# stateSpaceRobotics/pointcloud_obstacle_processing

Hardware: NVIDIA B200
Metric: points/sec per B200 job (HDL-64 120k-point frames: crop + 0.1 m voxel + RANSAC ground removal + Euclidean clustering + centroid/radius) (higher is better)
Workload: dtype f32

## Files before the change

pointcloud_obstacle_processing_b200/csrc/det_math.cuh:

```cuda
#pragma once
#include "common.cuh"

namespace pcop {

#define PCOP_INV_ODD_TABLE                                                                                            \
  {1.0 / 1.0,  1.0 / 3.0,  1.0 / 5.0,  1.0 / 7.0,  1.0 / 9.0,  1.0 / 11.0, 1.0 / 13.0, 1.0 / 15.0, 1.0 / 17.0, 1.0 / 19.0, \
   1.0 / 21.0, 1.0 / 23.0, 1.0 / 25.0, 1.0 / 27.0, 1.0 / 29.0}

__device__ inline double det_log(double x) {
  int e;
  double m = frexp(x, &e);
  if (m < 0.70710678118654752440) {
    m = dmul(m, 2.0);
    e -= 1;
  }
  const double s = ddiv(dsub(m, 1.0), dadd(m, 1.0));
  const double z = dmul(s, s);
  const double INV_ODD[15] = PCOP_INV_ODD_TABLE;
  double p = INV_ODD[14];
#pragma unroll
  for (int k = 13; k >= 0; --k) p = dadd(dmul(p, z), INV_ODD[k]);
  return dadd(dmul((double)e, 0.69314718055994530942), dmul(dmul(2.0, s), p));
}

__device__ inline double det_atan01(double t) {
  const double ATAN_K[5] = {0.0, 0.24497866312686415417, 0.46364760900080611621, 0.64350110879328438680,
                            0.78539816339744830962};
  const int k = (int)dadd(dmul(4.0, t), 0.5);
  const double c = dmul((double)k, 0.25);
  const double u = ddiv(dsub(t, c), dadd(1.0, dmul(t, c)));
  const double z = dmul(u, u);
  const double INV_ODD[15] = PCOP_INV_ODD_TABLE;
  double q = INV_ODD[10];
#pragma unroll
  for (int j = 9; j >= 0; --j) q = dsub(INV_ODD[j], dmul(z, q));
  return dadd(ATAN_K[k], dmul(u, q));
}

__device__ inline double det_atan2_ypos(double y, double x) {
  const double PI = 3.14159265358979323846, PI_2 = 1.57079632679489661923;
  if (y == 0.0) return (x >= 0.0) ? 0.0 : PI;
  if (x == 0.0) return PI_2;
  const double ax = fabs(x);
  double a;
  if (y <= ax) a = det_atan01(ddiv(y, ax));
  else a = dsub(PI_2, det_atan01(ddiv(ax, y)));
  return (x > 0.0) ? a : dsub(PI, a);
}

__device__ inline double det_sin(double x) {
  const double F[11] = {1.0,
                        1.0 / 6.0,
                        1.0 / 120.0,
                        1.0 / 5040.0,
                        1.0 / 362880.0,
                        1.0 / 39916800.0,
                        1.0 / 6227020800.0,
                        1.0 / 1307674368000.0,
                        1.0 / 355687428096000.0,
                        1.0 / 121645100408832000.0,
                        1.0 / 51090942171709440000.0};
  const double z = dmul(x, x);
  double p = 1.0 / 25852016738884976640000.0;
  for (int j = 10; j >= 0; --j) p = dsub(F[j], dmul(z, p));
  return dmul(x, p);
}

__device__ inline double det_cos(double x) {
  const double F[11] = {1.0,
                        1.0 / 2.0,
                        1.0 / 24.0,
                        1.0 / 720.0,
                        1.0 / 40320.0,
                        1.0 / 3628800.0,
                        1.0 / 479001600.0,
                        1.0 / 87178291200.0,
                        1.0 / 20922789888000.0,
                        1.0 / 6402373705728000.0,
                        1.0 / 2432902008176640000.0};
  const double z = dmul(x, x);
  double p = 1.0 / 1124000727777607680000.0;
  for (int j = 10; j >= 0; --j) p = dsub(F[j], dmul(z, p));
  return p;
}

__device__ inline double det_asin(double q) {
  if (q != q || fabs(q) > 1.0) return __longlong_as_double(0x7ff8000000000000ll);
  const double a = fabs(q);
  const double x = __dsqrt_rn(dmul(dsub(1.0, a), dadd(1.0, a)));
  const double r = det_atan2_ypos(a, x);
  return (q < 0.0) ? -r : r;
}

__device__ inline double det_tan(double x) { return ddiv(det_sin(x), det_cos(x)); }

}
```

pointcloud_obstacle_processing_b200/csrc/stage_plane.cu:

```cuda
#include "det_math.cuh"
#include <cstdio>
#include "internal.cuh"
#include "primitives.cuh"

namespace pcop {
#ifdef PCOP_PLANE_DEBUG_CLK
__device__ long long g_plane_loop_clk[16];
#define PL_CLK(k)                                                                  \
  do {                                                                             \
    if (blockIdx.y == 0 && rank == 0 && threadIdx.x == 0) g_plane_loop_clk[k] = clock64(); \
  } while (0)
#else
#define PL_CLK(k) \
  do {            \
  } while (0)
#endif

namespace {

constexpr int MAP_CAP = RNG_TABLE + 8;
constexpr double kHalfPi = 1.57079632679489661923;

__device__ __forceinline__ const float4* cur_cloud(const PlaneFrame& P, const float4* in, size_t in_stride,
                                                   float4* const* buf, int f, int cap) {
  return (P.cur < 0) ? (in + (size_t)f * in_stride) : (buf[P.cur] + (size_t)f * cap);
}

struct BufPair {
  float4* p[2];
  int* s[2];
};

__device__ bool model_valid(const PlaneConst& pc, const float4 co) {
  if (!(pc.eps_angle > 0.0)) return true;
  if (pc.eps_angle >= kHalfPi) return true;
  const double nx = co.x, ny = co.y, nz = co.z;
  const double dot = dadd(dadd(dmul(nx, pc.axis[0]), dmul(ny, pc.axis[1])), dmul(nz, pc.axis[2]));
  const double nn = __dsqrt_rn(dadd(dadd(dmul(nx, nx), dmul(ny, ny)), dmul(nz, nz)));
  const double na = __dsqrt_rn(dadd(dadd(dmul(pc.axis[0], pc.axis[0]), dmul(pc.axis[1], pc.axis[1])),
                                    dmul(pc.axis[2], pc.axis[2])));
  const double cosang = ddiv(fabs(dot), dmul(nn, na));
  return !(cosang < pc.cos_eps);
}

__device__ __forceinline__ bool collinear_ratio_test(const float4 p0, const float4 p1, const float4 p2) {
  const float ax = fdiv(fsub(p1.x, p0.x), fsub(p2.x, p0.x));
  const float ay = fdiv(fsub(p1.y, p0.y), fsub(p2.y, p0.y));
  const float az = fdiv(fsub(p1.z, p0.z), fsub(p2.z, p0.z));
  return (ax == ay) && (az == ay);
}

__device__ float4 compute_model(const float4 p0, const float4 p1, const float4 p2) {
  const float ax = fsub(p1.x, p0.x), ay = fsub(p1.y, p0.y), az = fsub(p1.z, p0.z);
  const float bx = fsub(p2.x, p0.x), by = fsub(p2.y, p0.y), bz = fsub(p2.z, p0.z);
  float nx = fsub(fmul(ay, bz), fmul(az, by));
  float ny = fsub(fmul(az, bx), fmul(ax, bz));
  float nz = fsub(fmul(ax, by), fmul(ay, bx));
  const float norm = __fsqrt_rn(fadd(fadd(fmul(nx, nx), fmul(ny, ny)), fmul(nz, nz)));
  nx = fdiv(nx, norm);
  ny = fdiv(ny, norm);
  nz = fdiv(nz, norm);
  const float d = -fadd(fadd(fmul(nx, p0.x), fmul(ny, p0.y)), fmul(nz, p0.z));
  return make_float4(nx, ny, nz, d);
}

__global__ void k_plane_init(PlaneFrame* __restrict__ pf, const int* __restrict__ n_in, double keep_fraction,
                             int* __restrict__ n_active, int* __restrict__ n_in_copy, int B) {
  const int f = blockIdx.x * blockDim.x + threadIdx.x;
  if (f >= B) return;
  PlaneFrame& P = pf[f];
  const int n = n_in[f];
  if (n_in_copy) n_in_copy[f] = n;
  P.cur = -1;
  P.nr_points = n;
  P.n = n;
  P.n_passes = 0;
  P.n_hyp = 0;
  P.gen_end = 0;
  P.best = -1;
  P.model_ok = 0;
  P.need_more = 0;
  P.n_inliers_last = 0;
  P.coeff_sel = make_float4(0.f, 0.f, 0.f, 0.f);
  P.coeff_ref = make_float4(0.f, 0.f, 0.f, 0.f);
  for (int k = 0; k < PCOP_MAX_PLANE_PASSES_RECORDED; ++k) {
    P.pass_points[k] = 0;
    P.pass_inliers[k] = 0;
    P.pass_coeff[k] = make_float4(0.f, 0.f, 0.f, 0.f);
  }
  P.active = ((double)n > dmul(keep_fraction, (double)n)) ? 1 : 0;
  if (P.active) atomicAdd(n_active, 1);
  atomicMax(n_active + 1, n);
  atomicAdd(n_active + 2, n);
}

// ... 171 lines not shown
        if (!gen_end) gen_end = 1;
        break;
      }
      const float4 co = compute_model(p0, p1, p2);
      if (lane == 0) {
        hyp[nh] = co;
        hyp_valid[nh] = model_valid(pc, co) ? 1 : 0;
      }
      ++nh;
    }
  }
  __syncwarp();
  nh_out = nh;
  gen_end_out = gen_end;
}

__global__ void __launch_bounds__(32)
    k_plane_gen(PlaneFrame* __restrict__ pf, const float4* __restrict__ in, size_t in_stride, BufPair bp,
                const int* __restrict__ rng, PlaneConst pc, uint32_t* __restrict__ warnings, int cap) {
  const int f = blockIdx.x;
  PlaneFrame& P = pf[f];
  if (!P.active) return;
  const int lane = threadIdx.x;
  __shared__ GenScratch G;
  int nh, gen_end;
  plane_gen_warp(cur_cloud(P, in, in_stride, bp.p, f, cap), P.n, rng, pc, G, P.hyp, P.hyp_valid, nh, gen_end);
  if (lane == 0) {
    P.n_hyp = nh;
    P.gen_end = gen_end;
    if (gen_end == 2) atomicOr(&warnings[f], (uint32_t)PCOP_WARN_RNG_TABLE_EXHAUSTED);
  }
  for (int h = lane; h < MAX_HYP; h += 32) P.counts[h] = 0;
}

__global__ void __launch_bounds__(CT_THREADS)
    k_plane_score(PlaneFrame* __restrict__ pf, const float4* __restrict__ in, size_t in_stride, BufPair bp, float thr,
                  int cap, int h_begin, int h_end, int second_phase) {
  const int f = blockIdx.y;
  PlaneFrame& P = pf[f];
  if (!P.active) return;
  if (second_phase && !P.need_more) return;
  const int n = P.n;
  if (blockIdx.x * CT_TILE >= n) return;
  const int nh = min(P.n_hyp, h_end);
  if (nh <= h_begin) return;
  __shared__ float4 hyp[MAX_HYP];
  __shared__ int cnt[MAX_HYP];
  if (threadIdx.x < MAX_HYP) {
    const float qnan = __uint_as_float(0x7fc00000u);
    hyp[threadIdx.x] = (threadIdx.x < nh) ? P.hyp[threadIdx.x] : make_float4(qnan, qnan, qnan, qnan);
    cnt[threadIdx.x] = 0;
  }
  __syncthreads();
  const float4* pts = cur_cloud(P, in, in_stride, bp.p, f, cap);
  const int lane = lane_id();
  for (int tile = blockIdx.x; tile * CT_TILE < n; tile += gridDim.x) {
  float4 p[CT_ITEMS];
#pragma unroll
  for (int k = 0; k < CT_ITEMS; ++k) {
    const int i = ct_index(tile, k);
    const float qnan = __uint_as_float(0x7fc00000u);
    p[k] = (i < n) ? __ldg(pts + i) : make_float4(qnan, qnan, qnan, qnan);
  }
  for (int h0 = h_begin; h0 < nh; h0 += 8) {
    int c[8];
#pragma unroll
    for (int j = 0; j < 8; ++j) {
      c[j] = 0;
      const float4 co = hyp[h0 + j];
#pragma unroll
      for (int k = 0; k < CT_ITEMS; ++k) c[j] += (plane_dist(co, p[k].x, p[k].y, p[k].z) < thr) ? 1 : 0;
    }
#pragma unroll
    for (int j = 0; j < 8; ++j) {
      const int s = __reduce_add_sync(FULL, c[j]);
      if (lane == 0 && s) atomicAdd(&cnt[h0 + j], s);
    }
  }
  }
  __syncthreads();
  if (threadIdx.x >= h_begin && threadIdx.x < nh && cnt[threadIdx.x]) atomicAdd(&P.counts[threadIdx.x], cnt[threadIdx.x]);
}

template <class CountFn>
__device__ __forceinline__ bool plane_select_replay(const PlaneConst& pc, double log_probability, int n, int nh, int navail,
                                                    const int* hyp_valid, CountFn count, int& sel_out) {
  const double one_over_indices = ddiv(1.0, (double)n);
  const double eps = 2.220446049250313e-16;
  int best = -2147483647;
  int sel = -1;
  double k = 1.0;
  for (int h = 0; h < nh; ++h) {
    if (!((double)h < k)) break;
    if (h >= navail) return true;
    const int c = hyp_valid[h] ? count(h) : 0;
    if (c > best) {
      best = c;
      sel = h;
      const double w = dmul((double)best, one_over_indices);
      double p_no = dsub(1.0, dmul(dmul(w, w), w));
      p_no = (eps < p_no) ? p_no : eps;
      p_no = (p_no < dsub(1.0, eps)) ? p_no : dsub(1.0, eps);
      k = ddiv(log_probability, det_log(p_no));
    }
    if (h + 1 > pc.max_iterations) break;
  }
  sel_out = sel;
  return false;
}

__global__ void k_plane_select(PlaneFrame* __restrict__ pf, PlaneConst pc, int B, int navail, int second_phase) {
  const int f = blockIdx.x * blockDim.x + threadIdx.x;
  if (f >= B) return;
  PlaneFrame& P = pf[f];
  if (!P.active) return;
  if (second_phase && !P.need_more) return;
  P.need_more = 0;
  int sel = -1;
  const int* counts = P.counts;
  if (plane_select_replay(pc, det_log(dsub(1.0, pc.probability)), P.n, P.n_hyp, navail, P.hyp_valid,
                          [counts](int h) { return counts[h]; }, sel)) {
    P.need_more = 1;
    return;
  }
  P.best = sel;
  P.model_ok = (sel >= 0 && P.hyp_valid[sel]) ? 1 : 0;
  P.coeff_sel = (sel >= 0) ? P.hyp[sel] : make_float4(0.f, 0.f, 0.f, 0.f);
  P.coeff_ref = P.coeff_sel;
}

template <int MINB>
__global__ void __launch_bounds__(256, MINB)
    k_plane_moments(const PlaneFrame* __restrict__ pf, const float4* __restrict__ in, size_t in_stride, BufPair bp,
                    float thr, double* __restrict__ partial, int chunks, int cap) {
  const int f = blockIdx.y, chunk = blockIdx.x;
  const PlaneFrame& P = pf[f];
  if (!P.active) return;
  const int n = P.n;
  if (chunk * TS_CHUNK >= n) return;
  const float4* pts = cur_cloud(P, in, in_stride, bp.p, f, cap);
  const float4 co = P.coeff_sel;
  const bool ok = P.model_ok != 0;
  double a[9];
#pragma unroll
  for (int k = 0; k < 9; ++k) a[k] = 0.0;
  int cnt = 0;
#pragma unroll
  for (int r = 0; r < TS_CHUNK / 256; ++r) {
    const int i = chunk * TS_CHUNK + r * 256 + threadIdx.x;
    double e[9];
#pragma unroll
    for (int k = 0; k < 9; ++k) e[k] = 0.0;
    if (i < n) {
      const float4 p = __ldg(pts + i);
      if (ok && plane_dist(co, p.x, p.y, p.z) < thr) {
        const double x = p.x, y = p.y, z = p.z;
        e[0] = dmul(x, x);
        e[1] = dmul(x, y);
        e[2] = dmul(x, z);
        e[3] = dmul(y, y);
        e[4] = dmul(y, z);
        e[5] = dmul(z, z);
        e[6] = x;
        e[7] = y;
        e[8] = z;
        ++cnt;
      }
    }
#pragma unroll
    for (int k = 0; k < 9; ++k) a[k] = dadd(a[k], e[k]);
  }
  __shared__ double sh[8][9];
  __shared__ int shc[8];
#pragma unroll
  for (int k = 0; k < 9; ++k) a[k] = tree_butterfly(a[k]);
  cnt = __reduce_add_sync(FULL, cnt);
  if (lane_id() == 0) {
#pragma unroll
    for (int k = 0; k < 9; ++k) sh[warp_id()][k] = a[k];
    shc[warp_id()] = cnt;
  }
  __syncthreads();
  double* out = partial + ((size_t)f * chunks + chunk) * 10;
  if (threadIdx.x < 9) {
    double s = sh[0][threadIdx.x];
    for (int w = 1; w < 8; ++w) s = dadd(s, sh[w][threadIdx.x]);
    out[threadIdx.x] = s;
  } else if (threadIdx.x == 9) {
    int c = 0;
    for (int w = 0; w < 8; ++w) c += shc[w];
    out[9] = (double)c;
  }
}

__device__ void compute_roots2(double b, double c, double* r) {
  r[0] = 0.0;
  double d = dsub(dmul(b, b), dmul(4.0, c));
  if (d < 0.0) d = 0.0;
  const double sd = __dsqrt_rn(d);
  r[2] = dmul(0.5, dadd(b, sd));
  r[1] = dmul(0.5, dsub(b, sd));
}

__device__ void compute_roots(const double* m, double* r) {
// ... 168 lines not shown
    if (i < n) {
      const float4 p = __ldg(pts + i);
      const bool inl = ok && plane_dist(co, p.x, p.y, p.z) < thr;
      if (!inl) keepmask |= 1u << k;
    }
  }
  unsigned wbase;
  const unsigned incl_total = big_tile_scan<BT_ITEMS>(keepmask, desc + (size_t)f * tiles, tile, sm, wbase);
#pragma unroll
  for (int k = 0; k < BT_ITEMS; ++k) {
    const int i = bt_index<BT_ITEMS>(tile, k);
    const bool keep = (keepmask >> k) & 1u;
    const unsigned m = __ballot_sync(FULL, keep);
    const unsigned pos = wbase + __popc(m & lanemask_lt());
    if (keep) {
      dpts[pos] = __ldg(pts + i);
      dsrc[pos] = srcidx ? srcidx[i] : i;
    } else if (i < n && inlier_idx) {
      inlier_idx[(size_t)f * cap + (i - (int)pos)] = i;
    }
    wbase += __popc(m);
  }
  if ((tile + 1) * BT_TILE >= n && threadIdx.x == 0) n_tmp[f] = (int)incl_total;
}

__global__ void k_plane_update(PlaneFrame* __restrict__ pf, const int* __restrict__ n_tmp, double keep_fraction,
                               int* __restrict__ n_active, uint32_t* __restrict__ warnings, int B) {
  const int f = blockIdx.x * blockDim.x + threadIdx.x;
  if (f >= B) return;
  PlaneFrame& P = pf[f];
  if (!P.active) {
    atomicMax(n_active + 1, P.n);
    atomicAdd(n_active + 2, P.n);
    return;
  }
  const int remaining = n_tmp[f];
  const int inliers = P.n - remaining;
  P.n_inliers_last = inliers;
  if (inliers == 0) {
    P.active = 0;
    atomicOr(&warnings[f], (uint32_t)PCOP_WARN_PLANE_BREAK);
    atomicMax(n_active + 1, P.n);
    atomicAdd(n_active + 2, P.n);
    return;
  }
  if (P.n_passes < PCOP_MAX_PLANE_PASSES_RECORDED) {
    P.pass_points[P.n_passes] = P.n;
    P.pass_inliers[P.n_passes] = inliers;
    P.pass_coeff[P.n_passes] = P.coeff_ref;
  }
  P.n_passes += 1;
  P.cur = (P.cur < 0) ? 0 : (1 - P.cur);
  P.n = remaining;
  P.active = ((double)remaining > dmul(keep_fraction, (double)P.nr_points)) ? 1 : 0;
  if (P.active) atomicAdd(n_active, 1);
  atomicMax(n_active + 1, P.n);
  atomicAdd(n_active + 2, P.n);
}

__global__ void __launch_bounds__(CT_THREADS)
    k_plane_finalize(const PlaneFrame* __restrict__ pf, const float4* __restrict__ in, size_t in_stride, BufPair bp,
                     float4* __restrict__ out, int* __restrict__ out_src, int* __restrict__ n_out, int cap) {
  const int f = blockIdx.y, tile = blockIdx.x;
  const PlaneFrame& P = pf[f];
  const int n = P.n;
  if (tile == 0 && threadIdx.x == 0) n_out[f] = n;
  if (tile * CT_TILE >= n) return;
  const float4* pts = cur_cloud(P, in, in_stride, bp.p, f, cap);
  const int* srcidx = (P.cur < 0) ? nullptr : (bp.s[P.cur] + (size_t)f * cap);
#pragma unroll
  for (int k = 0; k < CT_ITEMS; ++k) {
    const int i = ct_index(tile, k);
    if (i < n) {
      out[(size_t)f * cap + i] = __ldg(pts + i);
      out_src[(size_t)f * cap + i] = srcidx ? srcidx[i] : i;
    }
  }
}


constexpr int PL_CL = 8;
constexpr int PL_MAX_THREADS = 1024;
constexpr int PL_MAX_WARPS = PL_MAX_THREADS / 32;
constexpr int PL_MAX_GROUPS = PL_MAX_THREADS / 256;
constexpr int PL_N_BATCHES = 3;
__constant__ const int PL_BATCH_END[PL_N_BATCHES] = {4, 8, MAX_HYP};

struct PlShared {
  float4 hyp[MAX_HYP];
  int hyp_valid[MAX_HYP];
  int cnt[MAX_HYP];
  int cnt_all[PL_CL][MAX_HYP];
  int kept_all[PL_CL];
  int warp_excl[PL_MAX_WARPS];
  double msh[PL_MAX_GROUPS][8][9];
  int mcnt[PL_MAX_GROUPS][8];
  double log_prob;
  float4 coeff_sel, coeff_ref;
  int model_ok, need_more, nh, gen_end;
};

template <int GROUPS>
__device__ __forceinline__ void group_bar_sync(int g) {
  if (g == 0) asm volatile("bar.sync 1, 256;" ::: "memory");
  else if (g == 1) asm volatile("bar.sync 2, 256;" ::: "memory");
  else if (GROUPS > 2 && g == 2) asm volatile("bar.sync 3, 256;" ::: "memory");
  else if (GROUPS > 2) asm volatile("bar.sync 4, 256;" ::: "memory");
}
__device__ __forceinline__ unsigned cluster_ctarank() {
  unsigned r;
  asm volatile("mov.u32 %0, %%cluster_ctarank;" : "=r"(r));
  return r;
}
__device__ __forceinline__ void cluster_sync_all() {
  asm volatile("barrier.cluster.arrive.release.aligned;\n\tbarrier.cluster.wait.acquire.aligned;" ::: "memory");
}
template <class T>
__device__ __forceinline__ T* dsmem_ptr(T* p, unsigned rank) {
  unsigned long long out;
  asm volatile("mapa.u64 %0, %1, %2;" : "=l"(out) : "l"((unsigned long long)p), "r"(rank));
  return reinterpret_cast<T*>(out);
}

__global__ void __launch_bounds__(32)
    k_plane_gen0(PlaneFrame* __restrict__ pf, const float4* __restrict__ in, size_t in_stride, const int* __restrict__ n_in,
                 int* __restrict__ n_in_copy, const int* __restrict__ rng, PlaneConst pc, uint32_t* __restrict__ warnings) {
  const int f = blockIdx.x;
  const int lane = threadIdx.x;
  PlaneFrame& P = pf[f];
  const int n = n_in[f];
  const int active = ((double)n > dmul(pc.keep_fraction, (double)n)) ? 1 : 0;
  if (lane == 0) {
    if (n_in_copy) n_in_copy[f] = n;
    P.cur = -1;
    P.nr_points = n;
    P.n = n;
    P.n_passes = 0;
    P.best = -1;
    P.model_ok = 0;
    P.need_more = 0;
    P.n_inliers_last = 0;
    P.coeff_sel = make_float4(0.f, 0.f, 0.f, 0.f);
    P.coeff_ref = make_float4(0.f, 0.f, 0.f, 0.f);
    P.active = active;
  }
  if (lane == 1) P.log_prob = det_log(dsub(1.0, pc.probability));
  for (int k = lane; k < PCOP_MAX_PLANE_PASSES_RECORDED; k += 32) {
    P.pass_points[k] = 0;
    P.pass_inliers[k] = 0;
    P.pass_coeff[k] = make_float4(0.f, 0.f, 0.f, 0.f);
  }
  int nh = 0, gen_end = 0;
  if (active) {
    __shared__ GenScratch G;
    plane_gen_warp(in + (size_t)f * in_stride, n, rng, pc, G, P.hyp, P.hyp_valid, nh, gen_end);
  }
  if (lane == 0) {
    P.n_hyp = nh;
    P.gen_end = gen_end;
    if (gen_end == 2) atomicOr(&warnings[f], (uint32_t)PCOP_WARN_RNG_TABLE_EXHAUSTED);
  }
}

template <int G, int THREADS>
__device__ __forceinline__ void pl_score(PlShared& S, const float* __restrict__ sx, const float* __restrict__ sy,
                                         const float* __restrict__ sz, int sn, float thr, int h_begin, int h_end) {
  const int lane = threadIdx.x & 31;
  for (int h0 = h_begin; h0 < h_end; h0 += G) {
    int c[G];
    float4 co[G];
#pragma unroll
    for (int j = 0; j < G; ++j) {
      c[j] = 0;
      co[j] = S.hyp[h0 + j];
    }
    for (int i = threadIdx.x; i < sn; i += THREADS) {
      const float x = sx[i], y = sy[i], z = sz[i];
#pragma unroll
      for (int j = 0; j < G; ++j) c[j] += (plane_dist(co[j], x, y, z) < thr) ? 1 : 0;
    }
#pragma unroll
    for (int j = 0; j < G; ++j) {
      const int s = __reduce_add_sync(FULL, c[j]);
      if (lane == 0 && s) atomicAdd(&S.cnt[h0 + j], s);
    }
  }
}

template <int THREADS>
__device__ __forceinline__ void pl_push_counts(PlShared& S, unsigned rank, int h_begin, int h_end) {
  const int nhh = h_end - h_begin;
  for (int k = threadIdx.x; k < PL_CL * nhh; k += THREADS) {
    const unsigned r = (unsigned)(k / nhh);
    const int h = h_begin + k % nhh;
    *dsmem_ptr(&S.cnt_all[rank][h], r) = S.cnt[h];
  }
}

__device__ __forceinline__ void pl_select(PlShared& S, const PlaneConst& pc, int n, int navail) {
  int sel = -1;
  const PlShared* Sp = &S;
  const bool more = plane_select_replay(pc, S.log_prob, n, S.nh, navail, S.hyp_valid,
                                        [Sp](int h) {
                                          int c = 0;
#pragma unroll
                                          for (int r = 0; r < PL_CL; ++r) c += Sp->cnt_all[r][h];
                                          return c;
                                        },
                                        sel);
  S.need_more = more ? 1 : 0;
  if (more) return;
  S.model_ok = (sel >= 0 && S.hyp_valid[sel]) ? 1 : 0;
  S.coeff_sel = (sel >= 0) ? S.hyp[sel] : make_float4(0.f, 0.f, 0.f, 0.f);
  S.coeff_ref = S.coeff_sel;
}

template <int THREADS>
__global__ void __cluster_dims__(PL_CL, 1, 1) __launch_bounds__(THREADS, THREADS == 512 ? 2 : 1)
    k_plane_loop(PlaneFrame* __restrict__ pf, const float4* __restrict__ in, size_t in_stride, BufPair bp, PlaneConst pc,
                 const int* __restrict__ rng, int* __restrict__ inlier_idx, float4* __restrict__ out,
                 int* __restrict__ out_src, int* __restrict__ n_out, uint32_t* __restrict__ warnings, int cap,
                 int slice_cap, int nch_max, int n_lo, int n_hi) {
  constexpr int PL_THREADS = THREADS, PL_WARPS = THREADS / 32, PL_GROUPS = THREADS / 256;
  const unsigned rank = cluster_ctarank();
  const int f = blockIdx.y;
  const int tid = threadIdx.x, lane = tid & 31, warp = tid >> 5;
  extern __shared__ __align__(16) unsigned char pl_smem[];
  PlShared& S = *reinterpret_cast<PlShared*>(pl_smem);
  double* part = reinterpret_cast<double*>(pl_smem + sizeof(PlShared));
  float* sx = reinterpret_cast<float*>(pl_smem + sizeof(PlShared) + (size_t)nch_max * 80);
  float* sy = sx + slice_cap;
  float* sz = sy + slice_cap;
  GenScratch& G = *reinterpret_cast<GenScratch*>(sx);

  PlaneFrame& P = pf[f];
  int n = P.n, cur = P.cur, active = P.active, n_passes = P.n_passes;
  const int nr = P.nr_points;
  if (n <= n_lo || n > n_hi) return;
  bool first = true;

  if (!active) {
    const float4* pts = in + (size_t)f * in_stride;
    for (int i = (int)rank * PL_THREADS + tid; i < n; i += PL_CL * PL_THREADS) {
      out[(size_t)f * cap + i] = __ldg(pts + i);
      out_src[(size_t)f * cap + i] = i;
    }
    if (rank == 0 && tid == 0) n_out[f] = n;
    return;
  }

  while (true) {
    PL_CLK(0);
    const float4* pts = (cur < 0) ? (in + (size_t)f * in_stride) : (bp.p[cur] + (size_t)f * cap);
    const int* srcidx = (cur < 0) ? nullptr : (bp.s[cur] + (size_t)f * cap);
    const int SL = min(slice_cap, cdiv(cdiv(n, PL_CL), TS_CHUNK) * TS_CHUNK);
    const int lo = min((int)rank * SL, n), hi = min(lo + SL, n), sn = hi - lo;
    {
      const bool fresh = !first;
      for (int i0 = tid; i0 < sn; i0 += 8 * PL_THREADS) {
        float4 p[8];
#pragma unroll
        for (int u = 0; u < 8; ++u) {
          const int i = i0 + u * PL_THREADS;
          p[u] = (i < sn) ? (fresh ? __ldcg(pts + lo + i) : __ldg(pts + lo + i)) : make_float4(0.f, 0.f, 0.f, 0.f);
        }
#pragma unroll
        for (int u = 0; u < 8; ++u) {
          const int i = i0 + u * PL_THREADS;
          if (i < sn) {
            sx[i] = p[u].x;
            sy[i] = p[u].y;
            sz[i] = p[u].z;
          }
        }
      }
    }
    if (first) {
      if (tid == 0) {
        S.nh = P.n_hyp;
        S.gen_end = P.gen_end;
        S.log_prob = P.log_prob;
      }
      if (tid < MAX_HYP) {
        S.hyp[tid] = P.hyp[tid];
        S.hyp_valid[tid] = P.hyp_valid[tid];
      }
      first = false;
    }
    __syncthreads();
    if (tid < MAX_HYP) {
      const float qnan = __uint_as_float(0x7fc00000u);
      if (tid >= S.nh) S.hyp[tid] = make_float4(qnan, qnan, qnan, qnan);
      S.cnt[tid] = 0;
    }
    __syncthreads();
    const int nh = S.nh;
    PL_CLK(1);

    for (int ph = 0, scored = 0; ph < PL_N_BATCHES; ++ph) {
      const int end = PL_BATCH_END[ph];
      if (end - scored <= 4) pl_score<4, PL_THREADS>(S, sx, sy, sz, sn, pc.thr, scored, min(nh, end));
      else pl_score<8, PL_THREADS>(S, sx, sy, sz, sn, pc.thr, scored, min(nh, end));
      __syncthreads();
      pl_push_counts<PL_THREADS>(S, rank, scored, end);
      PL_CLK(2);
      cluster_sync_all();
      PL_CLK(3);
      if (tid == 0) pl_select(S, pc, n, end);
      __syncthreads();
      PL_CLK(4);
      if (!S.need_more) break;
      scored = end;
    }
    const bool ok = S.model_ok != 0;
    PL_CLK(5);

    if (pc.optimize && ok) {
      const float4 co = S.coeff_sel;
      const int g = tid >> 8, t = tid & 255, gw = (tid >> 5) & 7;
      const int nlc = cdiv(sn, TS_CHUNK);
      const int gc0 = lo / TS_CHUNK;
      for (int lc = g; lc < nlc; lc += PL_GROUPS) {
        double a[9];
#pragma unroll
        for (int k = 0; k < 9; ++k) a[k] = 0.0;
        int cnt = 0;
#pragma unroll
        for (int r = 0; r < TS_CHUNK / 256; ++r) {
          const int i = lc * TS_CHUNK + r * 256 + t;
          double e[9];
#pragma unroll
          for (int k = 0; k < 9; ++k) e[k] = 0.0;
          if (i < sn) {
            const float px = sx[i], py = sy[i], pz = sz[i];
            if (plane_dist(co, px, py, pz) < pc.thr) {
              const double x = px, y = py, z = pz;
              e[0] = dmul(x, x);
              e[1] = dmul(x, y);
              e[2] = dmul(x, z);
              e[3] = dmul(y, y);
              e[4] = dmul(y, z);
              e[5] = dmul(z, z);
              e[6] = x;
              e[7] = y;
              e[8] = z;
              ++cnt;
            }
          }
#pragma unroll
          for (int k = 0; k < 9; ++k) a[k] = dadd(a[k], e[k]);
        }
#pragma unroll
        for (int k = 0; k < 9; ++k) a[k] = tree_butterfly(a[k]);
        cnt = __reduce_add_sync(FULL, cnt);
        if (lane == 0) {
#pragma unroll
          for (int k = 0; k < 9; ++k) S.msh[g][gw][k] = a[k];
          S.mcnt[g][gw] = cnt;
        }
        group_bar_sync<PL_GROUPS>(g);
        double* o = part + (size_t)(gc0 + lc) * 10;
        if (t < 9) {
          double s = S.msh[g][0][t];
          for (int w = 1; w < 8; ++w) s = dadd(s, S.msh[g][w][t]);
          o[t] = s;
        } else if (t == 9) {
          int c = 0;
          for (int w = 0; w < 8; ++w) c += S.mcnt[g][w];
          o[9] = (double)c;
        }
        group_bar_sync<PL_GROUPS>(g);
      }
      __syncthreads();
      const int nv = nlc * 10;
      for (int k = tid; k < (PL_CL - 1) * nv; k += PL_THREADS) {
        const unsigned r = (rank + 1u + (unsigned)(k / nv)) % PL_CL;
        double* mine = part + (size_t)gc0 * 10 + k % nv;
        *dsmem_ptr(mine, r) = *mine;
      }
      PL_CLK(6);
      cluster_sync_all();
      PL_CLK(7);
      if (warp == 0) {
        const int nch = cdiv(n, TS_CHUNK);
        double tot = 0.0;
        if (lane < 10)
          for (int c = 0; c < nch; ++c) tot = dadd(tot, part[(size_t)c * 10 + lane]);
        double a[9];
#pragma unroll
        for (int k = 0; k < 9; ++k) a[k] = __shfl_sync(FULL, tot, k);
        const double cntd = __shfl_sync(FULL, tot, 9);
        if (lane == 0) {
          float4 o;
          if (plane_refine_model(pc, a, cntd, o)) S.coeff_ref = o;
        }
      }
      __syncthreads();
    }

    PL_CLK(8);
    const float4 co = S.coeff_ref;
    const int per_warp = cdiv(cdiv(sn, PL_WARPS), 32) * 32;
    const int rows = per_warp / 32;
    const int wb = warp * per_warp;
    unsigned keepmask = 0u;
    for (int r = 0; r < rows; ++r) {
      const int i = wb + r * 32 + lane;
      if (i < sn) {
        const bool inl = ok && plane_dist(co, sx[i], sy[i], sz[i]) < pc.thr;
        if (!inl) keepmask |= 1u << r;
      }
    }
    const unsigned wtotal = __reduce_add_sync(FULL, (unsigned)__popc(keepmask));
    if (lane == 0) S.warp_excl[warp] = (int)wtotal;
    __syncthreads();
    if (warp == 0) {
      const int v = (lane < PL_WARPS) ? S.warp_excl[lane] : 0;
      int incl = v;
#pragma unroll
      for (int o = 1; o < 32; o <<= 1) {
        const int up = __shfl_up_sync(FULL, incl, o);
        if (lane >= o) incl += up;
      }
      if (lane < PL_WARPS) S.warp_excl[lane] = incl - v;
      const int total = __shfl_sync(FULL, incl, 31);
      if (lane < PL_CL) *dsmem_ptr(&S.kept_all[rank], (unsigned)lane) = total;
    }
    PL_CLK(9);
    cluster_sync_all();
    PL_CLK(10);
    int base = 0, remaining = 0;
#pragma unroll
    for (int r = 0; r < PL_CL; ++r) {
      const int k = S.kept_all[r];
      base += (r < (int)rank) ? k : 0;
      remaining += k;
    }
    const int inliers = n - remaining;
    const bool go_on = inliers != 0 && ((double)remaining > dmul(pc.keep_fraction, (double)nr));
    const int dst = (cur < 0) ? 0 : (1 - cur);
    float4* dpts = go_on ? (bp.p[dst] + (size_t)f * cap) : (out + (size_t)f * cap);
    int* dsrc = go_on ? (bp.s[dst] + (size_t)f * cap) : (out_src + (size_t)f * cap);
    unsigned wbase = (unsigned)(base + S.warp_excl[warp]);
    for (int r = 0; r < rows; ++r) {
      const int i = wb + r * 32 + lane;
      const bool keep = (keepmask >> r) & 1u;
      const unsigned m = __ballot_sync(FULL, keep);
      const unsigned pos = wbase + __popc(m & lanemask_lt());
      const int gi = lo + i;
      if (keep) {
        dpts[pos] = __ldcg(pts + gi);
        dsrc[pos] = srcidx ? __ldcg(srcidx + gi) : gi;
      } else if (i < sn && inlier_idx) {
        inlier_idx[(size_t)f * cap + (gi - (int)pos)] = gi;
      }
      wbase += __popc(m);
    }

    PL_CLK(11);
    if (inliers == 0) {
      if (rank == 0 && tid == 0) {
        P.n_inliers_last = 0;
        P.active = 0;
        P.coeff_sel = S.coeff_sel;
        P.coeff_ref = S.coeff_ref;
        atomicOr(&warnings[f], (uint32_t)PCOP_WARN_PLANE_BREAK);
        n_out[f] = n;
      }
      return;
    }
    if (rank == 0 && tid == 0) {
      if (n_passes < PCOP_MAX_PLANE_PASSES_RECORDED) {
        P.pass_points[n_passes] = n;
        P.pass_inliers[n_passes] = inliers;
        P.pass_coeff[n_passes] = S.coeff_ref;
      }
      P.n_passes = n_passes + 1;
      P.n_inliers_last = inliers;
      P.n = remaining;
      P.coeff_sel = S.coeff_sel;
      P.coeff_ref = S.coeff_ref;
      P.active = go_on ? 1 : 0;
      if (!go_on) n_out[f] = remaining;
    }
    if (!go_on) return;
    n_passes += 1;
    cur = dst;
    n = remaining;

    __threadfence();
    cluster_sync_all();
    if (warp == 0) {
      int gnh, gen_end;
      plane_gen_warp(bp.p[cur] + (size_t)f * cap, n, rng, pc, G, S.hyp, S.hyp_valid, gnh, gen_end);
      if (lane == 0) {
        S.nh = gnh;
        S.gen_end = gen_end;
        if (gen_end == 2 && rank == 0) atomicOr(&warnings[f], (uint32_t)PCOP_WARN_RNG_TABLE_EXHAUSTED);
      }
    }
    __syncthreads();
  }
}

}

constexpr int PL_SLICE_MAX = 16384;
constexpr int PL_SLICE_SMALL = 8192;
constexpr int PL_RESIDENT_MAX = PL_CL * PL_SLICE_MAX;

static cudaError_t run_plane_hostloop(const Ctx& c, const PlaneArgs& a);
static void run_plane_finalize(const Ctx& c, const PlaneArgs& a, float4* out, int* out_src);

int plane_small_tier_max() { return PL_CL * PL_SLICE_SMALL; }
int plane_resident_max() { return PL_RESIDENT_MAX; }

cudaError_t run_plane(const Ctx& c, const PlaneArgs& a) {
  if (!a.resident) {
    const cudaError_t e = run_plane_hostloop(c, a);
    if (e != cudaSuccess) return e;
    run_plane_finalize(c, a, a.out, a.out_src);
    return cudaGetLastError();
  }
  BufPair bp;
  bp.p[0] = a.buf[0];
  bp.p[1] = a.buf[1];
  bp.s[0] = a.src[0];
  bp.s[1] = a.src[1];
  KL(c, "k_plane_gen0", k_plane_gen0<<<c.B, 32, 0, c.stream>>>(a.pf, a.in, a.in_stride, a.n_in, a.n_in_copy, a.rng, a.pc, a.warnings));
  count_launch(c);
  static_assert(sizeof(GenScratch) <= 4096 * 12, "the generator scratch overlays the smallest slice planes");
  static_assert(sizeof(PlShared) % 16 == 0, "alignment of the regions behind PlShared");
  auto smem_bytes = [](int slice_cap) { return sizeof(PlShared) + (size_t)(PL_CL * slice_cap / TS_CHUNK) * 80 + (size_t)slice_cap * 12; };
  const int bound = std::min(c.grid_cap, PL_RESIDENT_MAX);
  const int small_slice = std::min(PL_SLICE_SMALL, std::max(4096, cdiv(cdiv(bound, PL_CL), TS_CHUNK) * TS_CHUNK));
  const int small_max = PL_CL * small_slice;
  {
    const size_t smem = smem_bytes(small_slice);
    cudaFuncSetAttribute(k_plane_loop<512>, cudaFuncAttributeMaxDynamicSharedMemorySize, (int)smem);
    KL(c, "k_plane_loop", k_plane_loop<512><<<dim3(PL_CL, c.B), 512, smem, c.stream>>>(
                              a.pf, a.in, a.in_stride, bp, a.pc, a.rng, a.inlier_idx, a.out, a.out_src, a.n_out, a.warnings,
                              c.cap, small_slice, PL_CL * small_slice / TS_CHUNK, -1, small_max));
    count_launch(c);
  }
  if (c.grid_cap > small_max && a.large_tier) {
    const int slice_cap = cdiv(cdiv(bound, PL_CL), TS_CHUNK) * TS_CHUNK;
    const size_t smem = smem_bytes(slice_cap);
    cudaFuncSetAttribute(k_plane_loop<1024>, cudaFuncAttributeMaxDynamicSharedMemorySize, (int)smem);
    KL(c, "k_plane_loop_large", k_plane_loop<1024><<<dim3(PL_CL, c.B), 1024, smem, c.stream>>>(
                                    a.pf, a.in, a.in_stride, bp, a.pc, a.rng, a.inlier_idx, a.out, a.out_src, a.n_out,
                                    a.warnings, c.cap, slice_cap, PL_CL * slice_cap / TS_CHUNK, small_max, PL_RESIDENT_MAX));
    count_launch(c);
  }
  return cudaGetLastError();
}

static cudaError_t run_plane_hostloop(const Ctx& c, const PlaneArgs& a) {
  const int tiles = cdiv(c.cap, CT_TILE);
  const int gtiles = cdiv(c.grid_cap, CT_TILE);
  const int chunks = cdiv(c.cap, TS_CHUNK);
  const int gchunks = cdiv(c.grid_cap, TS_CHUNK);
  BufPair bp;
  bp.p[0] = a.buf[0];
  bp.p[1] = a.buf[1];
  bp.s[0] = a.src[0];
  bp.s[1] = a.src[1];
  cudaError_t e;
  cudaMemsetAsync(a.n_active, 0, 3 * sizeof(int), c.stream);
  KL(c, "k_plane_init", k_plane_init<<<cdiv(c.B, 128), 128, 0, c.stream>>>(a.pf, a.n_in, a.pc.keep_fraction, a.n_active, a.n_in_copy, c.B));
  count_launch(c);
  cudaMemcpyAsync(a.h_n_active, a.n_active, 3 * sizeof(int), cudaMemcpyDeviceToHost, c.stream);
  if ((e = cudaStreamSynchronize(c.stream)) != cudaSuccess) return e;
  Ctx cc = c;
  while (*a.h_n_active > 0) {
    cc.grid_cap = max(1, min(c.grid_cap, a.h_n_active[1]));
    const int gtiles = cdiv(cc.grid_cap, CT_TILE);
    const int gchunks = cdiv(cc.grid_cap, TS_CHUNK);
    KL(c, "k_plane_gen", k_plane_gen<<<c.B, 32, 0, c.stream>>>(a.pf, a.in, a.in_stride, bp, a.rng, a.pc, a.warnings, c.cap));
    constexpr int PHASE1 = 8;
    KL(c, "k_plane_score", k_plane_score<<<dim3(gtiles, c.B), CT_THREADS, 0, c.stream>>>(a.pf, a.in, a.in_stride, bp, a.pc.thr, c.cap, 0, PHASE1, 0));
    KL(c, "k_plane_select", k_plane_select<<<cdiv(c.B, 128), 128, 0, c.stream>>>(a.pf, a.pc, c.B, PHASE1, 0));
    KL(c, "k_plane_score", k_plane_score<<<dim3(std::min(gtiles, 8), c.B), CT_THREADS, 0, c.stream>>>(a.pf, a.in, a.in_stride, bp, a.pc.thr, c.cap, PHASE1, MAX_HYP, 1));
    KL(c, "k_plane_select", k_plane_select<<<cdiv(c.B, 128), 128, 0, c.stream>>>(a.pf, a.pc, c.B, MAX_HYP, 1));
    KL(c, "k_plane_moments", k_plane_moments<4><<<dim3(gchunks, c.B), 256, 0, c.stream>>>(a.pf, a.in, a.in_stride, bp, a.pc.thr,
                                                                                          a.partial, chunks, c.cap));
    KL(c, "k_plane_refine", k_plane_refine<<<c.B, 32, 0, c.stream>>>(a.pf, a.partial, a.pc, chunks));
    const int btiles = cdiv(c.cap, BT_TILE), gbtiles = cdiv(cc.grid_cap, BT_TILE);
    cudaMemsetAsync(a.desc, 0, (size_t)c.B * btiles * sizeof(unsigned), c.stream);
    KL(c, "k_plane_extract", k_plane_extract<8><<<dim3(c.B, gbtiles), CT_THREADS, 0, c.stream>>>(
                                 a.pf, a.in, a.in_stride, bp, a.pc.thr, a.inlier_idx, a.n_tmp, a.desc, c.cap, btiles));
    cudaMemsetAsync(a.n_active, 0, 3 * sizeof(int), c.stream);
    KL(c, "k_plane_update", k_plane_update<<<cdiv(c.B, 128), 128, 0, c.stream>>>(a.pf, a.n_tmp, a.pc.keep_fraction, a.n_active, a.warnings, c.B));
    count_launch(c, 9);
    cudaMemcpyAsync(a.h_n_active, a.n_active, 3 * sizeof(int), cudaMemcpyDeviceToHost, c.stream);
    if ((e = cudaStreamSynchronize(c.stream)) != cudaSuccess) return e;
  }
  return cudaGetLastError();
}

static void run_plane_finalize(const Ctx& c, const PlaneArgs& a, float4* out, int* out_src) {
  const int tiles = cdiv(c.cap, CT_TILE);
  const int gtiles = cdiv(c.grid_cap, CT_TILE);
  BufPair bp;
  bp.p[0] = a.buf[0];
  bp.p[1] = a.buf[1];
  bp.s[0] = a.src[0];
  bp.s[1] = a.src[1];
  KL(c, "k_plane_finalize", k_plane_finalize<<<dim3(gtiles, c.B), CT_THREADS, 0, c.stream>>>(a.pf, a.in, a.in_stride, bp, out, out_src, a.n_out,
                                                                  c.cap));
  count_launch(c);
}

}

#ifdef PCOP_PLANE_DEBUG_CLK
extern "C" int pcop_debug_plane_loop_cycles(long long* out16) {
  return (int)cudaMemcpyFromSymbol(out16, pcop::g_plane_loop_clk, sizeof(long long) * 16);
}
#endif
```

Measured before the change: 22.35 billion.

## Fuse first-batch plane scoring into slice load and parallelize hypothesis selection

Scores the first four RANSAC hypotheses while points are loaded into shared-memory slices, which drops a separate scoring pass for the first batch. Hypothesis selection now runs on a whole warp: each lane computes counts and adaptive-k values for its hypotheses in parallel, and a shuffle-based replay replaces the serial single-thread log computations. The moment reduction switches from group-partitioned named barriers to per-chunk shared arrays with a block barrier. The atan table becomes a select chain to avoid local memory, and the debug clock instrumentation is extended with per-block phase accumulation. Fusing the scoring adds register pressure to the load loop, and the shared-memory moment arrays grow.

```diff
diff --git a/pointcloud_obstacle_processing_b200/csrc/det_math.cuh b/pointcloud_obstacle_processing_b200/csrc/det_math.cuh
--- a/pointcloud_obstacle_processing_b200/csrc/det_math.cuh
+++ b/pointcloud_obstacle_processing_b200/csrc/det_math.cuh
@@ -24,8 +24,6 @@
 }
 
 __device__ inline double det_atan01(double t) {
-  const double ATAN_K[5] = {0.0, 0.24497866312686415417, 0.46364760900080611621, 0.64350110879328438680,
-                            0.78539816339744830962};
   const int k = (int)dadd(dmul(4.0, t), 0.5);
   const double c = dmul((double)k, 0.25);
   const double u = ddiv(dsub(t, c), dadd(1.0, dmul(t, c)));
@@ -34,7 +32,12 @@
   double q = INV_ODD[10];
 #pragma unroll
   for (int j = 9; j >= 0; --j) q = dsub(INV_ODD[j], dmul(z, q));
-  return dadd(ATAN_K[k], dmul(u, q));
+  const double atan_k = (k == 0)   ? 0.0
+                        : (k == 1) ? 0.24497866312686415417
+                        : (k == 2) ? 0.46364760900080611621
+                        : (k == 3) ? 0.64350110879328438680
+                                   : 0.78539816339744830962;
+  return dadd(atan_k, dmul(u, q));
 }
 
 __device__ inline double det_atan2_ypos(double y, double x) {
diff --git a/pointcloud_obstacle_processing_b200/csrc/stage_plane.cu b/pointcloud_obstacle_processing_b200/csrc/stage_plane.cu
--- a/pointcloud_obstacle_processing_b200/csrc/stage_plane.cu
+++ b/pointcloud_obstacle_processing_b200/csrc/stage_plane.cu
@@ -5,12 +5,25 @@
 
 namespace pcop {
 #ifdef PCOP_PLANE_DEBUG_CLK
-__device__ long long g_plane_loop_clk[16];
-#define PL_CLK(k)                                                                  \
-  do {                                                                             \
-    if (blockIdx.y == 0 && rank == 0 && threadIdx.x == 0) g_plane_loop_clk[k] = clock64(); \
+constexpr int PL_DBG_SLOTS = 12, PL_DBG_ROWS = 8192;
+__device__ unsigned long long g_plane_phase[PL_DBG_ROWS][PL_DBG_SLOTS];
+__device__ unsigned g_plane_phase_rows;
+#define PL_CLK_INIT()                                                  \
+  long long pl_t_prev = clock64();                                     \
+  unsigned pl_row = PL_DBG_ROWS;                                       \
+  if (threadIdx.x == 0) pl_row = atomicAdd(&g_plane_phase_rows, 1u)
+#define PL_CLK(k)                                                                             \
+  do {                                                                                        \
+    if (threadIdx.x == 0 && pl_row < PL_DBG_ROWS) {                                           \
+      const long long t_ = clock64();                                                         \
+      atomicAdd(&g_plane_phase[pl_row][k], (unsigned long long)(t_ - pl_t_prev));             \
+      pl_t_prev = t_;                                                                         \
+    }                                                                                         \
   } while (0)
 #else
+#define PL_CLK_INIT() \
+  do {                \
+  } while (0)
 #define PL_CLK(k) \
   do {            \
   } while (0)
@@ -348,11 +361,18 @@
   if (threadIdx.x >= h_begin && threadIdx.x < nh && cnt[threadIdx.x]) atomicAdd(&P.counts[threadIdx.x], cnt[threadIdx.x]);
 }
 
-template <class CountFn>
-__device__ __forceinline__ bool plane_select_replay(const PlaneConst& pc, double log_probability, int n, int nh, int navail,
-                                                    const int* hyp_valid, CountFn count, int& sel_out) {
-  const double one_over_indices = ddiv(1.0, (double)n);
+__device__ __forceinline__ double adaptive_k(double log_probability, double one_over_indices, int count) {
   const double eps = 2.220446049250313e-16;
+  const double w = dmul((double)count, one_over_indices);
+  double p_no = dsub(1.0, dmul(dmul(w, w), w));
+  p_no = (eps < p_no) ? p_no : eps;
+  p_no = (p_no < dsub(1.0, eps)) ? p_no : dsub(1.0, eps);
+  return ddiv(log_probability, det_log(p_no));
+}
+
+template <class CountFn, class KFn>
+__device__ __forceinline__ bool plane_select_replay(const PlaneConst& pc, int nh, int navail, const int* hyp_valid,
+                                                    CountFn count, KFn k_of, int& sel_out) {
   int best = -2147483647;
   int sel = -1;
   double k = 1.0;
@@ -363,11 +383,7 @@
     if (c > best) {
       best = c;
       sel = h;
-      const double w = dmul((double)best, one_over_indices);
-      double p_no = dsub(1.0, dmul(dmul(w, w), w));
-      p_no = (eps < p_no) ? p_no : eps;
-      p_no = (p_no < dsub(1.0, eps)) ? p_no : dsub(1.0, eps);
-      k = ddiv(log_probability, det_log(p_no));
+      k = k_of(h, best);
     }
     if (h + 1 > pc.max_iterations) break;
   }
@@ -384,8 +400,9 @@
   P.need_more = 0;
   int sel = -1;
   const int* counts = P.counts;
-  if (plane_select_replay(pc, det_log(dsub(1.0, pc.probability)), P.n, P.n_hyp, navail, P.hyp_valid,
-                          [counts](int h) { return counts[h]; }, sel)) {
+  const double log_probability = det_log(dsub(1.0, pc.probability)), one_over_indices = ddiv(1.0, (double)P.n);
+  if (plane_select_replay(pc, P.n_hyp, navail, P.hyp_valid, [counts](int h) { return counts[h]; },
+                          [=](int, int c) { return adaptive_k(log_probability, one_over_indices, c); }, sel)) {
     P.need_more = 1;
     return;
   }
@@ -720,7 +737,8 @@
 constexpr int PL_CL = 8;
 constexpr int PL_MAX_THREADS = 1024;
 constexpr int PL_MAX_WARPS = PL_MAX_THREADS / 32;
-constexpr int PL_MAX_GROUPS = PL_MAX_THREADS / 256;
+constexpr int PL_SLICE_MAX = 16384;
+constexpr int PL_SLICE_CHUNKS = PL_SLICE_MAX / TS_CHUNK;
 constexpr int PL_N_BATCHES = 3;
 __constant__ const int PL_BATCH_END[PL_N_BATCHES] = {4, 8, MAX_HYP};
 
@@ -731,20 +749,13 @@
   int cnt_all[PL_CL][MAX_HYP];
   int kept_all[PL_CL];
   int warp_excl[PL_MAX_WARPS];
-  double msh[PL_MAX_GROUPS][8][9];
-  int mcnt[PL_MAX_GROUPS][8];
+  double msh[PL_SLICE_CHUNKS][8][9];
+  int mcnt[PL_SLICE_CHUNKS][8];
   double log_prob;
   float4 coeff_sel, coeff_ref;
   int model_ok, need_more, nh, gen_end;
 };
 
-template <int GROUPS>
-__device__ __forceinline__ void group_bar_sync(int g) {
-  if (g == 0) asm volatile("bar.sync 1, 256;" ::: "memory");
-  else if (g == 1) asm volatile("bar.sync 2, 256;" ::: "memory");
-  else if (GROUPS > 2 && g == 2) asm volatile("bar.sync 3, 256;" ::: "memory");
-  else if (GROUPS > 2) asm volatile("bar.sync 4, 256;" ::: "memory");
-}
 __device__ __forceinline__ unsigned cluster_ctarank() {
   unsigned r;
   asm volatile("mov.u32 %0, %%cluster_ctarank;" : "=r"(r));
@@ -836,16 +847,34 @@
 }
 
 __device__ __forceinline__ void pl_select(PlShared& S, const PlaneConst& pc, int n, int navail) {
+  static_assert(MAX_HYP <= 64, "two hypotheses per lane");
+  const int lane = threadIdx.x & 31;
+  const double one_over_indices = ddiv(1.0, (double)n);
+  int c[2] = {0, 0};
+  double kh[2] = {1.0, 1.0};
+#pragma unroll
+  for (int q = 0; q < 2; ++q) {
+    const int h = lane + 32 * q;
+    if (q == 1 && navail <= 32) break;
+    if (h < navail && h < S.nh && S.hyp_valid[h]) {
+#pragma unroll
+      for (int r = 0; r < PL_CL; ++r) c[q] += S.cnt_all[r][h];
+    }
+    kh[q] = adaptive_k(S.log_prob, one_over_indices, c[q]);
+  }
   int sel = -1;
-  const PlShared* Sp = &S;
-  const bool more = plane_select_replay(pc, S.log_prob, n, S.nh, navail, S.hyp_valid,
-                                        [Sp](int h) {
-                                          int c = 0;
-#pragma unroll
-                                          for (int r = 0; r < PL_CL; ++r) c += Sp->cnt_all[r][h];
-                                          return c;
-                                        },
-                                        sel);
+  const bool more = plane_select_replay(
+      pc, S.nh, navail, S.hyp_valid,
+      [&](int h) {
+        const int lo = __shfl_sync(FULL, c[0], h & 31), hi = __shfl_sync(FULL, c[1], h & 31);
+        return h < 32 ? lo : hi;
+      },
+      [&](int h, int) {
+        const double lo = __shfl_sync(FULL, kh[0], h & 31), hi = __shfl_sync(FULL, kh[1], h & 31);
+        return h < 32 ? lo : hi;
+      },
+      sel);
+  if (lane != 0) return;
   S.need_more = more ? 1 : 0;
   if (more) return;
   S.model_ok = (sel >= 0 && S.hyp_valid[sel]) ? 1 : 0;
@@ -887,14 +916,25 @@
     return;
   }
 
+  PL_CLK_INIT();
   while (true) {
     PL_CLK(0);
     const float4* pts = (cur < 0) ? (in + (size_t)f * in_stride) : (bp.p[cur] + (size_t)f * cap);
     const int* srcidx = (cur < 0) ? nullptr : (bp.s[cur] + (size_t)f * cap);
     const int SL = min(slice_cap, cdiv(cdiv(n, PL_CL), TS_CHUNK) * TS_CHUNK);
     const int lo = min((int)rank * SL, n), hi = min(lo + SL, n), sn = hi - lo;
+    int c[4];
     {
       const bool fresh = !first;
+      const float4* hsrc = first ? P.hyp : S.hyp;
+      const int nh0 = first ? P.n_hyp : S.nh;
+      const float qnan = __uint_as_float(0x7fc00000u);
+      float4 co[4];
+#pragma unroll
+      for (int j = 0; j < 4; ++j) {
+        co[j] = (j < nh0) ? hsrc[j] : make_float4(qnan, qnan, qnan, qnan);
+        c[j] = 0;
+      }
       for (int i0 = tid; i0 < sn; i0 += 8 * PL_THREADS) {
         float4 p[8];
 #pragma unroll
@@ -906,12 +946,16 @@
         for (int u = 0; u < 8; ++u) {
           const int i = i0 + u * PL_THREADS;
           if (i < sn) {
+#pragma unroll
+            for (int j = 0; j < 4; ++j) c[j] += (plane_dist(co[j], p[u].x, p[u].y, p[u].z) < pc.thr) ? 1 : 0;
             sx[i] = p[u].x;
             sy[i] = p[u].y;
             sz[i] = p[u].z;
           }
         }
       }
+#pragma unroll
+      for (int j = 0; j < 4; ++j) c[j] = __reduce_add_sync(FULL, c[j]);
     }
     if (first) {
       if (tid == 0) {
@@ -932,19 +976,25 @@
       S.cnt[tid] = 0;
     }
     __syncthreads();
+    if (lane == 0) {
+#pragma unroll
+      for (int j = 0; j < 4; ++j)
+        if (c[j]) atomicAdd(&S.cnt[j], c[j]);
+    }
     const int nh = S.nh;
     PL_CLK(1);
 
     for (int ph = 0, scored = 0; ph < PL_N_BATCHES; ++ph) {
       const int end = PL_BATCH_END[ph];
-      if (end - scored <= 4) pl_score<4, PL_THREADS>(S, sx, sy, sz, sn, pc.thr, scored, min(nh, end));
+      if (ph == 0) {
+      } else if (end - scored <= 4) pl_score<4, PL_THREADS>(S, sx, sy, sz, sn, pc.thr, scored, min(nh, end));
       else pl_score<8, PL_THREADS>(S, sx, sy, sz, sn, pc.thr, scored, min(nh, end));
       __syncthreads();
       pl_push_counts<PL_THREADS>(S, rank, scored, end);
       PL_CLK(2);
       cluster_sync_all();
       PL_CLK(3);
-      if (tid == 0) pl_select(S, pc, n, end);
+      if (warp == 0) pl_select(S, pc, n, end);
       __syncthreads();
       PL_CLK(4);
       if (!S.need_more) break;
@@ -993,21 +1043,23 @@
         cnt = __reduce_add_sync(FULL, cnt);
         if (lane == 0) {
 #pragma unroll
-          for (int k = 0; k < 9; ++k) S.msh[g][gw][k] = a[k];
-          S.mcnt[g][gw] = cnt;
+          for (int k = 0; k < 9; ++k) S.msh[lc][gw][k] = a[k];
+          S.mcnt[lc][gw] = cnt;
         }
-        group_bar_sync<PL_GROUPS>(g);
+      }
+      __syncthreads();
+      if (tid < nlc * 10) {
+        const int lc = tid / 10, k = tid % 10;
         double* o = part + (size_t)(gc0 + lc) * 10;
-        if (t < 9) {
-          double s = S.msh[g][0][t];
-          for (int w = 1; w < 8; ++w) s = dadd(s, S.msh[g][w][t]);
-          o[t] = s;
-        } else if (t == 9) {
+        if (k < 9) {
+          double s = S.msh[lc][0][k];
+          for (int w = 1; w < 8; ++w) s = dadd(s, S.msh[lc][w][k]);
+          o[k] = s;
+        } else {
           int c = 0;
-          for (int w = 0; w < 8; ++w) c += S.mcnt[g][w];
+          for (int w = 0; w < 8; ++w) c += S.mcnt[lc][w];
           o[9] = (double)c;
         }
-        group_bar_sync<PL_GROUPS>(g);
       }
       __syncthreads();
       const int nv = nlc * 10;
@@ -1143,7 +1195,6 @@
 
 }
 
-constexpr int PL_SLICE_MAX = 16384;
 constexpr int PL_SLICE_SMALL = 8192;
 constexpr int PL_RESIDENT_MAX = PL_CL * PL_SLICE_MAX;
 
@@ -1252,7 +1303,17 @@
 }
 
 #ifdef PCOP_PLANE_DEBUG_CLK
-extern "C" int pcop_debug_plane_loop_cycles(long long* out16) {
-  return (int)cudaMemcpyFromSymbol(out16, pcop::g_plane_loop_clk, sizeof(long long) * 16);
+extern "C" int pcop_debug_plane_phase_rows(long long* out, int max_rows) {
+  unsigned rows = 0;
+  if (cudaMemcpyFromSymbol(&rows, pcop::g_plane_phase_rows, sizeof(unsigned)) != cudaSuccess) return -1;
+  const int n = std::min<int>(std::min<unsigned>(rows, pcop::PL_DBG_ROWS), max_rows);
+  if (n > 0 && cudaMemcpyFromSymbol(out, pcop::g_plane_phase, sizeof(long long) * pcop::PL_DBG_SLOTS * n) != cudaSuccess)
+    return -1;
+  void* p;
+  if (cudaGetSymbolAddress(&p, pcop::g_plane_phase) != cudaSuccess || cudaMemset(p, 0, sizeof(pcop::g_plane_phase)) != cudaSuccess)
+    return -1;
+  const unsigned zero = 0;
+  if (cudaMemcpyToSymbol(pcop::g_plane_phase_rows, &zero, sizeof(unsigned)) != cudaSuccess) return -1;
+  return (int)std::min<unsigned>(rows, 0x7fffffffu);
 }
 #endif
```

New measurement: 22.44 billion, median of 6. About the same (+0.4%).
